# JingInAI/Quantize

Hardware: AMD Instinct MI355X
Metric: quant-conv2d images/sec at batch 256 (ResNet-50, W8A8) (higher is better)
Workload: dtype int8

## Files before the change

### quantize_amd/capi.py

```python
import contextlib
import ctypes
import os

from . import loader

_lib = None

QE_OK = 0
QE_ERR_UNSUPPORTED = 7
DTYPES = {"uint8": 0, "int8": 1, "int16": 2, "int32": 3, "int64": 4,
          "float16": 5, "float32": 6, "float64": 7}

ACTS = {None: 0, "none": 0, "gelu": 1}


class QeConvShape(ctypes.Structure):
    _fields_ = [(n, ctypes.c_int32) for n in ("N", "IC", "H", "W", "OC", "KH", "KW", "stride", "padding")]


class QeQParam(ctypes.Structure):
    _fields_ = [("data", ctypes.c_void_p), ("n_bits", ctypes.c_int32), ("sign", ctypes.c_int32),
                ("scale", ctypes.c_void_p), ("zero", ctypes.c_void_p), ("n_param", ctypes.c_int32)]


class QeRequant(ctypes.Structure):
    _fields_ = [("scale", ctypes.c_void_p), ("zero", ctypes.c_void_p), ("n_param", ctypes.c_int32),
                ("qmin", ctypes.c_float), ("qmax", ctypes.c_float), ("n_bits", ctypes.c_int32), ("sign", ctypes.c_int32)]


class QeError(RuntimeError):
    pass


_vp, _i32, _i64, _sz, _f32, _str = (ctypes.c_void_p, ctypes.c_int, ctypes.c_int64, ctypes.c_size_t, ctypes.c_float,
                                    ctypes.c_char_p)
_pq, _ps, _pr, _ppc = ctypes.POINTER(QeQParam), ctypes.POINTER(QeConvShape), ctypes.POINTER(QeRequant), ctypes.POINTER(_vp)
_attn = [_vp, _vp, _vp, _vp, _i32, _i32, _i32, _i32, _i32, _i64, _i64, _i64, _i64, _i64, _i64, _f32]

PROTOTYPES = {
    "qe_error_string": (_str, [_i32]),
    "qe_last_hip_error": (_i32, []),
    "qe_version": (_str, []),
    "qe_target_arch": (_str, []),
    "qe_packed_nbytes": (_i64, [_i64, _i32]),
    "qe_tpack": (_i32, [_vp, _i32, _i64, _i32, _i32, _vp, _vp, _vp]),
    "qe_tunpack": (_i32, [_vp, _i64, _i32, _i32, _vp, _vp]),
    "qe_quantize_pack": (_i32, [_vp, _i64, _vp, _vp, _i32, _i64, _f32, _f32, _i32, _i32, _vp, _vp, _vp]),
    "qe_quantize_pack_act": (_i32, [_vp, _i64, _i32, _vp, _vp, _i32, _i64, _f32, _f32, _i32, _i32, _vp, _vp, _vp, _vp]),
    "qe_quantize_patchify": (_i32, [_vp, _i32, _i32, _i32, _i32, _i32, _vp, _vp, _i32, _f32, _f32, _i32, _i32, _vp, _vp, _vp]),
    "qe_global_avgpool": (_i32, [_vp, _i64, _i32, _vp, _vp]),
    "qe_maxpool2d_codes": (_i32, [_vp, _i32, _i32, _i32, _i32, _i32, _i32, _i32, _vp, _vp]),
    "qe_quantconv2d_path": (_i32, [_ps, _pq, _pq]),
    "qe_quantconv2d_workspace_bytes": (_sz, [_ps, _i32, _i32]),
    "qe_quantconv2d": (_i32, [_pq, _pq, _vp, _ps, _vp, _vp, _sz, _vp]),
    "qe_conv_prepared_bytes": (_sz, [_ps, _i32, _i32]),
    "qe_conv_prepared_layout": (ctypes.c_uint64, [_ps, _i32, _i32]),
    "qe_conv_prepare": (_i32, [_pq, _vp, _ps, _i32, _vp, _sz, _vp]),
    "qe_quantconv2d_prepared_workspace_bytes": (_sz, [_ps, _i32, _i32]),
    "qe_quantconv2d_prepared": (_i32, [_pq, _pq, _vp, _ps, _vp, _sz, _vp, _vp, _sz, _vp]),
    "qe_quantconv2d_requant_path": (_i32, [_ps, _pq, _pq, _pr]),
    "qe_quantconv2d_requant_workspace_bytes": (_sz, [_ps, _pq, _pq, _pr]),
    "qe_quantconv2d_requant_prepared": (_i32, [_pq, _pq, _vp, _ps, _vp, _sz, _pr, _vp, _vp, _vp, _sz, _vp]),
    "qe_quantconv2d_residual_path": (_i32, [_ps, _pq, _pq, _pr]),
    "qe_quantconv2d_residual_workspace_bytes": (_sz, [_ps, _pq, _pq, _pr]),
    "qe_quantconv2d_residual_prepared": (_i32, [_pq, _pq, _vp, _ps, _vp, _sz, _vp, _vp, _pr, _vp, _vp, _vp, _sz, _vp]),
    "qe_quantconv2d_float_input": (_i32, [_vp, _pq, _vp, _ps, _vp, _vp]),
    "qe_quantconv2d_float_input_path": (_i32, [_ps, _pq]),
    "qe_quantconv2d_float_input_workspace_bytes": (_sz, [_ps, _i32]),
    "qe_quantconv2d_float_input_ws": (_i32, [_vp, _pq, _vp, _ps, _vp, _vp, _sz, _vp]),
    "qe_conv_f32_prepare": (_i32, [_pq, _vp, _ps, _vp, _sz, _vp]),
    "qe_quantconv2d_float_input_prepared": (_i32, [_vp, _pq, _vp, _ps, _vp, _sz, _vp, _vp]),
    "qe_quantlinear": (_i32, [_pq, _pq, _vp, _i64, _i32, _i32, _vp, _vp]),
    "qe_quantlinear_path": (_i32, [_pq, _pq, _i64, _i32, _i32]),
    "qe_quantlinear_form": (_i32, [_pq, _pq, _i64, _i32, _i32, _i32]),
    "qe_quantlinear_float_input": (_i32, [_vp, _pq, _vp, _i64, _i32, _i32, _vp, _vp]),
    "qe_quantlinear_float_input_path": (_i32, [_vp, _pq, _i64, _i32, _i32]),
    "qe_quantlinear_requant_path": (_i32, [_pq, _pq, _i64, _i32, _i32, _pr, _vp]),
    "qe_quantlinear_requant_workspace_bytes": (_sz, [_pq, _pq, _i64, _i32, _i32, _pr, _vp]),
    "qe_quantlinear_requant": (_i32, [_pq, _pq, _vp, _i64, _i32, _i32, _i32, _pr, _vp, _vp, _vp, _sz, _vp]),
    "qe_quantlinear_residual_path": (_i32, [_pq, _pq, _i64, _i32, _i32]),
    "qe_quantlinear_residual_workspace_bytes": (_sz, [_pq, _pq, _i64, _i32, _i32]),
    "qe_quantlinear_residual": (_i32, [_pq, _pq, _vp, _i64, _i32, _i32, _vp, _vp, _vp, _sz, _vp]),
    "qe_quantlinear_float_input_residual_path": (_i32, [_vp, _pq, _i64, _i32, _i32]),
    "qe_quantlinear_float_input_residual_workspace_bytes": (_sz, [_vp, _pq, _i64, _i32, _i32]),
    "qe_quantlinear_float_input_residual": (_i32, [_vp, _pq, _vp, _i64, _i32, _i32, _vp, _vp, _vp, _sz, _vp]),
    "qe_layernorm_quantize_pack_path": (_i32, [_i64, _i32, _i32, _pr, _ppc]),
    "qe_layernorm_quantize_pack_workspace_bytes": (_sz, [_i64, _i32, _i32, _pr, _ppc, _vp]),
    "qe_layernorm_quantize_pack": (_i32, [_vp, _i64, _i32, _vp, _vp, _f32, _i32, _pr, _ppc, _vp, _vp, _vp, _sz, _vp]),
    "qe_attention_path": (_i32, [_i32, _i32, _i32, _i32]),
    "qe_attention": (_i32, _attn + [_vp]),
    "qe_attention_masked_path": (_i32, [_i32, _i32, _i32, _i32, _i32, _i32, _i32]),
    "qe_attention_masked": (_i32, _attn + [_vp, _i64, _i64, _vp, _i32, _vp]),
}
SYMBOLS = sorted(PROTOTYPES)
DEBUG_PROTOTYPES = {
    "qe_debug_reload_env": (None, []),
    "qe_debug_set_stamp_buffer": (None, [_vp]),
}


def lib():
    global _lib
    if _lib is not None:
        return _lib
    path = os.environ.get("QE_LIB") or loader.lib_path()
    if not os.path.exists(path):
        raise ImportError("libqe_hip.so not built: run `python -m quantize_amd.build`. No fallback exists.")
    L = ctypes.CDLL(path)
    for table in (PROTOTYPES, DEBUG_PROTOTYPES):
        for name, (restype, argtypes) in table.items():
            f = getattr(L, name)
            f.restype, f.argtypes = restype, argtypes
    _lib = L
    return L


def check(rc):
    if rc != QE_OK:
        L = lib()
        msg = L.qe_error_string(rc).decode()
        if rc == 5:
            msg += " (hipError_t %d)" % L.qe_last_hip_error()
        raise QeError(msg)


def _stream(stream=None):
    import torch
    s = torch.cuda.current_stream() if stream is None else stream
    return ctypes.c_void_p(s.cuda_stream)


def _ptr(t):
    return None if t is None else t.data_ptr()


def _ws(need, dev):
    import torch
    return torch.empty(need, dtype=torch.uint8, device=dev) if need else None


def _status(status, dev):
    import torch
    return torch.zeros(1, dtype=torch.int32, device=dev) if status is None else status


def _prep(t):
    return (t.data_ptr(), t.numel()) if t is not None and t.numel() else (None, 0)


def packed_nbytes(n, n_bits):
    return int(lib().qe_packed_nbytes(int(n), int(n_bits)))


def tpack(x, n_bits, sign, out=None, status=None, stream=None):
    import torch
    assert x.is_cuda and x.is_contiguous()
    n = x.numel()
    if out is None:
        out = torch.empty(packed_nbytes(n, n_bits), dtype=torch.uint8, device=x.device)
    status = _status(status, x.device)
    check(lib().qe_tpack(x.data_ptr(), DTYPES[str(x.dtype).replace("torch.", "")], n, int(n_bits),
                         1 if sign else 0, out.data_ptr(), status.data_ptr(), _stream(stream)))
    return out, status


def tunpack(packed, n, n_bits, sign, out=None, stream=None):
    import torch
    assert packed.is_cuda and packed.is_contiguous() and packed.dtype == torch.uint8
    if out is None:
        out = torch.empty(n, dtype=torch.int8 if sign else torch.uint8, device=packed.device)
    check(lib().qe_tunpack(packed.data_ptr(), int(n), int(n_bits), 1 if sign else 0, out.data_ptr(),
                           _stream(stream)))
    return out


def conv_shape(N, IC, H, W, OC, KH, KW, stride, padding):
    return QeConvShape(int(N), int(IC), int(H), int(W), int(OC), int(KH), int(KW), int(stride), int(padding))


def out_hw(sh):
# ... 413 lines not shown
```

### quantize_amd/csrc/qe_api.hip

```cpp
#include "qe_common.h"
#include "qe_conv_plan.hpp"

#include <atomic>
#include <cstring>
#include <mutex>
#include <string>
#include <utility>
#include <vector>
#include <unistd.h>

extern char **environ;

namespace qe {

thread_local int g_last_hip_error = 0;

namespace {
struct EnvSnapshot {
    std::vector<std::pair<std::string, std::string>> kv;
};
std::atomic<EnvSnapshot *> g_env{nullptr};
std::mutex g_env_mutex;
EnvSnapshot *take_env_snapshot()
{
// ... 31 lines not shown
                               uint8_t *codes, int32_t *status, hipStream_t s);

static int check_shape(const qe_conv_shape *sh)
{
    if (sh == nullptr) return QE_ERR_ARG;
    if (sh->N < 0 || sh->IC <= 0 || sh->H <= 0 || sh->W <= 0 || sh->OC < 0 || sh->KH <= 0 || sh->KW <= 0 ||
        sh->stride <= 0 || sh->padding < 0)
        return QE_ERR_ARG;
    return QE_OK;
}

static int check_nparam(const qe_qparam *x, const qe_qparam *w, const qe_conv_shape *sh)
{
    if (x != nullptr && !(x->n_param == 1 || x->n_param >= sh->IC)) return QE_ERR_ARG;
    if (!(w->n_param == 1 || w->n_param >= sh->OC)) return QE_ERR_ARG;
    return QE_OK;
}

static int check_qparam(const qe_qparam *q)
{
    if (q == nullptr || q->data == nullptr || q->scale == nullptr || q->zero == nullptr) return QE_ERR_ARG;
    if (!(q->n_bits > 0 && q->n_bits <= 8)) return QE_ERR_NBITS;
    if (q->n_param < 1) return QE_ERR_ARG;
    return QE_OK;
}

static int check_packed_conv(const qe_conv_shape *sh, const qe_qparam *x, const qe_qparam *w)
{
    int rc = check_shape(sh);
    if (rc != QE_OK) return rc;
    if ((rc = check_qparam(x)) != QE_OK) return rc;
    if ((rc = check_qparam(w)) != QE_OK) return rc;
    return check_nparam(x, w, sh);
}

}

extern "C" const char *qe_error_string(int status)
{
    switch (status) {
        case QE_OK: return "ok";
        case QE_ERR_NBITS: return "n_bits must be in the range (0, 8]";
        case QE_ERR_RANGE: return "The input tensor is out of range.";
        case QE_ERR_DTYPE: return "unsupported element type";
        case QE_ERR_ARG: return "invalid argument";
        case QE_ERR_HIP: return "HIP runtime error";
        case QE_ERR_WORKSPACE: return "workspace too small";
        case QE_ERR_UNSUPPORTED: return "problem shape not supported by the gfx950 kernels";
        default: return "unknown error";
    }
}

extern "C" int qe_last_hip_error(void) { return qe::g_last_hip_error; }

extern "C" void qe_debug_reload_env(void)
{
    std::lock_guard<std::mutex> lock(qe::g_env_mutex);
    qe::g_env.store(qe::take_env_snapshot(), std::memory_order_release);
}
extern "C" const char *qe_version(void) { return "quantize_amd 0.1.0"; }
extern "C" const char *qe_target_arch(void) { return "gfx950"; }

namespace qe {
static ConvPlan plan_bits(const qe_conv_shape *sh, int x_bits, int w_bits)
{
    qe_qparam x{}, w{};
    x.n_bits = x_bits; x.n_param = 1;
    w.n_bits = w_bits; w.n_param = 1;
    return plan_conv({sh, &x, &w});
}
static size_t scratch_bytes(const ConvPlan &p) { return (p.m.total - p.m.prep_total + 255) / 256 * 256; }
}

extern "C" size_t qe_quantconv2d_workspace_bytes(const qe_conv_shape *shape, int x_bits, int w_bits)
{
    if (qe::check_shape(shape) != QE_OK) return 0;
    return qe::plan_bits(shape, x_bits, w_bits).m.total;
}

extern "C" int qe_quantconv2d_path(const qe_conv_shape *shape, const qe_qparam *x, const qe_qparam *w)
{
    if (qe::check_shape(shape) != QE_OK || x == nullptr || w == nullptr) return 0;
    return qe::plan_conv({shape, x, w}).route != qe::ConvRoute::Generic ? 1 : 0;
}

extern "C" int qe_quantconv2d(const qe_qparam *x, const qe_qparam *w, const float *bias,
                              const qe_conv_shape *shape, float *out,
                              void *workspace, size_t workspace_bytes, qe_stream_t stream)
{
    using namespace qe;
    const int rc = check_packed_conv(shape, x, w);
    if (rc != QE_OK) return rc;
    if (out == nullptr) return QE_ERR_ARG;
    hipStream_t s = static_cast<hipStream_t>(stream);
    const ConvPlan p = plan_conv({shape, x, w, reinterpret_cast<uintptr_t>(out)});
    if (p.route == ConvRoute::Generic) return launch_conv_generic(true, x->data, x, w, bias, shape, out, s);
    return launch_conv_mfma(p, x, w, bias, shape, out, workspace, workspace_bytes, nullptr, 0, false, s, nullptr, nullptr);
}

extern "C" size_t qe_conv_prepared_bytes(const qe_conv_shape *shape, int x_bits, int w_bits)
{
    if (qe::check_shape(shape) != QE_OK) return 0;
    return qe::plan_prepared(shape, x_bits, w_bits).prep_total;
}

extern "C" uint64_t qe_conv_prepared_layout(const qe_conv_shape *shape, int x_bits, int w_bits)
{
    if (qe::check_shape(shape) != QE_OK) return 0;
    return qe::prepared_layout(qe::plan_prepared(shape, x_bits, w_bits), shape);
}

extern "C" size_t qe_quantconv2d_prepared_workspace_bytes(const qe_conv_shape *shape, int x_bits, int w_bits)
{
    if (qe::check_shape(shape) != QE_OK) return 0;
    const qe::ConvPlan p = qe::plan_bits(shape, x_bits, w_bits);
    return p.m.total - p.m.prep_total;
}

extern "C" int qe_conv_prepare(const qe_qparam *w, const float *bias, const qe_conv_shape *shape, int x_bits,
                               void *prepared, size_t prepared_bytes, qe_stream_t stream)
{
    using namespace qe;
    int rc = check_shape(shape);
    if (rc != QE_OK) return rc;
    if ((rc = check_qparam(w)) != QE_OK) return rc;
    if ((rc = check_nparam(nullptr, w, shape)) != QE_OK) return rc;
    if (!(x_bits > 0 && x_bits <= 8)) return QE_ERR_NBITS;
    return prepare_conv_tables(plan_prepared(shape, x_bits, w->n_bits), w, bias, shape, prepared, prepared_bytes,
                               static_cast<hipStream_t>(stream));
}

extern "C" int qe_quantconv2d_prepared(const qe_qparam *x, const qe_qparam *w, const float *bias,
                                       const qe_conv_shape *shape, const void *prepared, size_t prepared_bytes,
                                       float *out, void *workspace, size_t workspace_bytes, qe_stream_t stream)
{
    using namespace qe;
    const int rc = check_packed_conv(shape, x, w);
    if (rc != QE_OK) return rc;
    if (out == nullptr) return QE_ERR_ARG;
    hipStream_t s = static_cast<hipStream_t>(stream);
    const ConvPlan p = plan_conv({shape, x, w, reinterpret_cast<uintptr_t>(out)});
    if (p.route == ConvRoute::Generic)
        return launch_conv_generic(true, x->data, x, w, bias, shape, out, s);
    return launch_conv_mfma(p, x, w, bias, shape, out, workspace, workspace_bytes, prepared, prepared_bytes, true, s, nullptr,
                            nullptr);
}

static int check_requant(const qe_requant *rq)
{
    if (rq == nullptr || rq->scale == nullptr || rq->zero == nullptr) return QE_ERR_ARG;
    if (!(rq->n_bits > 0 && rq->n_bits <= 8)) return QE_ERR_NBITS;
    if (rq->n_param < 1) return QE_ERR_ARG;
    return QE_OK;
}

static qe::ConvPlan plan_requant(const qe_conv_shape *shape, const qe_qparam *x, const qe_qparam *w, const qe_requant *rq,
                                 const uint8_t *out)
{
    qe::ConvRequest r{shape, x, w};
    r.rq_out = reinterpret_cast<uintptr_t>(out);
    r.rq_bits = rq->n_bits;
    r.rq_n_param = rq->n_param;
    return qe::plan_conv(r);
}

extern "C" int qe_quantconv2d_requant_path(const qe_conv_shape *shape, const qe_qparam *x, const qe_qparam *w, const qe_requant *rq)
// ... 271 lines not shown
```

### quantize_amd/csrc/qe_conv_flatd.hip

```cpp
#include "qe_conv_mfma_kernel.hpp"
#include "qe_conv_plan.hpp"

#include <utility>

namespace qe {

struct FlatdArgs {
    const uint8_t *x;
    const uint8_t *w;
    const float *x_scale, *x_zero, *w_scale, *w_zero, *bias;
    int x_sign, w_sign, w_per_tensor;
    float *out;
    int N, IC, OC, P;
    int tiles_per_image;
    int n_pix_tiles, n_oc_tiles, chunk;
    uint8_t *rq_out;
    const float *rq_scale, *rq_zero;
    float rq_qmin, rq_qmax, rq_lo, rq_hi;
    unsigned rq_offset;
    int32_t *rq_status;
};

constexpr int FD_RING_DEFAULT = 3;

// ... 227 lines not shown
        for (int t = 0; t < NT; ++t) {
            const int v = sxacc[t] + __shfl_xor(sxacc[t], 32);
            if (h == 0) sxp[32 * t + col] = v;
        }
    }
    __syncthreads();
    if constexpr (RQ) {
        uint8_t *bp = smem + wave * (32 * 49 * 4);
        const int oc0 = ot * FD_MT + wave * 32;
        RqConst rqc = rq_setup(a);
        rqc.slow = __builtin_amdgcn_readfirstlane(rqc.slow);
        rqc.chk = __builtin_amdgcn_readfirstlane(rqc.chk);
        bool bad = false;
        const bool fast = rq_fast_ok(rqc) && __builtin_amdgcn_ballot_w64(!rq_bounded(alpha, cst, bia, zwp)) == 0ull;
#pragma unroll
        for (int gi = 0; gi < 4; ++gi) {
            const bool img = n0 + gi < a.N;
#pragma unroll
            for (int tt = 0; tt < 2; ++tt) {
#pragma unroll
                for (int r = 0; r < 16; r += 2) {
                    const int pxl = 32 * tt + (r & 3) + 8 * (r >> 2) + 4 * h;
                    float f0 = (float)acc[2 * gi + tt][r] + cst, f1 = (float)acc[2 * gi + tt][r + 1] + cst;
                    if (need_sx) {
                        f0 = fmaf(-zwp, (float)sxp[64 * gi + pxl], f0);
                        f1 = fmaf(-zwp, (float)sxp[64 * gi + pxl + 1], f1);
                    }
                    const float y0 = fmaf(alpha, f0, bia), y1 = fmaf(alpha, f1, bia);
                    float c0, c1;
                    if (fast) {
                        const v2f c2 = rq_fast2(rqc, v2f{y0, y1});
                        c0 = c2.x; c1 = c2.y;
                    } else {
                        bool b0 = false, b1 = false;
                        c0 = rq_value(rqc, y0, b0);
                        c1 = rq_value(rqc, y1, b1);
                        bad |= img && oc < a.OC && ((b0 && pxl < P) || (b1 && pxl + 1 < P));
                    }
                    if (pxl < P) bp[col * P + pxl] = (uint8_t)(unsigned)c0;
                    if (pxl + 1 < P) bp[col * P + pxl + 1] = (uint8_t)(unsigned)c1;
                }
            }
            if (img && oc0 + 32 <= a.OC) {
                uint8_t *dst = a.rq_out + ((int64_t)(n0 + gi) * a.OC + oc0) * P;
#pragma unroll
                for (int k = 0; k < 2; ++k) {
                    const uint4 d4 = *reinterpret_cast<const uint4 *>(bp + 16 * (64 * k + lane));
                    if (64 * k + lane < 98) *reinterpret_cast<uint4 *>(dst + 16 * (64 * k + lane)) = d4;
                }
            }
        }
        rq_report(a, bad);
    } else {
        float *patch = reinterpret_cast<float *>(smem) + wave * (32 * 49);
        const int oc0 = ot * FD_MT + wave * 32;
        const int vrows = min(32, a.OC - oc0);
        const int nfl = vrows > 0 ? vrows * P : 0;
        const bool vec_ok = (reinterpret_cast<uintptr_t>(a.out) & 15) == 0;
#pragma unroll
        for (int gi = 0; gi < 4; ++gi) {
#pragma unroll
            for (int tt = 0; tt < 2; ++tt) {
#pragma unroll
                for (int r = 0; r < 16; ++r) {
                    const int pxl = 32 * tt + (r & 3) + 8 * (r >> 2) + 4 * h;
                    float f = (float)acc[2 * gi + tt][r] + cst;
                    if (need_sx) f = fmaf(-zwp, (float)sxp[64 * gi + pxl], f);
                    if (pxl < P) patch[col * P + pxl] = fmaf(alpha, f, bia);
                }
            }
            __builtin_amdgcn_s_waitcnt(0xc07f);
            if (n0 + gi < a.N) {
                float *dst = a.out + ((int64_t)(n0 + gi) * a.OC + oc0) * P;
                for (int i = lane; 4 * i < nfl; i += 64) {
                    if (vec_ok && 4 * i + 4 <= nfl) *reinterpret_cast<float4 *>(dst + 4 * i) = *reinterpret_cast<const float4 *>(patch + 4 * i);
                    else for (int b = 4 * i; b < nfl && b < 4 * i + 4; ++b) dst[b] = patch[b];
                }
            }
            __builtin_amdgcn_s_waitcnt(0xc07f);
        }
    }
}

int launch_flatd(const ConvPlan &p, const qe_qparam *x, const qe_qparam *w, const float *bias, float *out, hipStream_t s,
                 const RequantHost *rq)
{
    const qe_conv_shape *sh = &p.run;
    FlatdArgs a;
    a.rq_out = nullptr; a.rq_scale = nullptr; a.rq_zero = nullptr; a.rq_status = nullptr;
    a.rq_qmin = a.rq_qmax = a.rq_lo = a.rq_hi = 0.0f; a.rq_offset = 0;
    if (rq != nullptr) {
        a.rq_out = rq->out; a.rq_scale = rq->scale; a.rq_zero = rq->zero;
        a.rq_qmin = rq->qmin; a.rq_qmax = rq->qmax; a.rq_status = rq->status;
        a.rq_offset = rq->sign ? 128u : 0u;
        a.rq_lo = rq->sign ? -128.0f : 0.0f; a.rq_hi = rq->sign ? 127.0f : 255.0f;
    }
    a.x = static_cast<const uint8_t *>(x->data); a.w = static_cast<const uint8_t *>(w->data);
    a.x_scale = x->scale; a.x_zero = x->zero; a.w_scale = w->scale; a.w_zero = w->zero; a.bias = bias;
    a.x_sign = x->sign; a.w_sign = w->sign; a.w_per_tensor = (w->n_param == 1);
    a.out = out; a.N = sh->N; a.IC = sh->IC; a.OC = sh->OC; a.P = sh->H * sh->W;
    a.n_oc_tiles = p.n_oc_tiles;
    a.tiles_per_image = p.tiles_h;
    a.n_pix_tiles = p.n_pix_tiles;
    a.chunk = p.chunk;
    const int64_t blocks = p.blocks;
#define QE_FD_LAUNCH(WV, RQ)                                                                                                \
    do {                                                                                                                    \
        static const bool ok_ = hipFuncSetAttribute(reinterpret_cast<const void *>(&conv_flatd_kernel<3, WV, RQ>),          \
                                                    hipFuncAttributeMaxDynamicSharedMemorySize, FdGeom<3, WV>::LDS) == hipSuccess; \
        (void)ok_;                                                                                                          \
        constexpr size_t lds_ = FdGeom<3, WV>::LDS;                                                                         \
        hipLaunchKernelGGL((conv_flatd_kernel<3, WV, RQ>), dim3((unsigned)blocks), dim3(64 * WV), lds_, s, a);              \
    } while (0)
    if (rq != nullptr) {
        if (p.fd_w8) QE_FD_LAUNCH(8, true); else QE_FD_LAUNCH(4, true);
    } else {
        if (p.fd_w8) QE_FD_LAUNCH(8, false); else QE_FD_LAUNCH(4, false);
    }
#undef QE_FD_LAUNCH
    QE_LAUNCH_CHECK();
    return QE_OK;
}

}
```

### quantize_amd/csrc/qe_conv_plan.hip

```cpp
#include "qe_conv_plan.hpp"
#include "qe_conv_mfma_kernel.hpp"

#include <algorithm>
#include <cstdlib>

namespace qe {

static int knob(const char *name, int dflt)
{
    const char *e = env_get(name);
    return e ? atoi(e) : dflt;
}

static size_t align_up(size_t v, size_t a) { return (v + a - 1) / a * a; }

static const int kNiw[3][3] = {{7, 4, 2}, {4, 2, 1}, {2, 1, 0}};
static const int kWN[3] = {1, 2, 4};

static MfmaPlan make_plan8(const qe_conv_shape *sh, int w_bits, bool x4 = false)
{
    MfmaPlan p;
    p.OH = (sh->H + 2 * sh->padding - sh->KH) / sh->stride + 1;
    p.OW = (sh->W + 2 * sh->padding - sh->KW) / sh->stride + 1;
    p.KK = sh->KH * sh->KW;
// ... 221 lines not shown
    return p;
}

MfmaPlan plan_prepared(const qe_conv_shape *sh, int x_bits, int w_bits)
{
    qe_conv_shape s1 = *sh;
    const int64_t img = (int64_t)sh->IC * sh->H * sh->W;
    s1.N = img >= 64 ? 1 : (int)((64 + img - 1) / img);
    return make_plan(&s1, x_bits, w_bits);
}

uint64_t prepared_layout(const MfmaPlan &p, const qe_conv_shape *sh)
{
    if (!p.ok || p.prep_total == 0) return 0;
    uint64_t h = 1469598103934665603ull;
    auto mix = [&](uint64_t v) { h = (h ^ v) * 1099511628211ull; };
    mix(p.smallic ? 1 : 0); mix((uint64_t)p.OCP); mix((uint64_t)p.NG); mix((uint64_t)p.KK); mix((uint64_t)sh->KH); mix((uint64_t)sh->KW);
    mix((uint64_t)sh->IC); mix((uint64_t)sh->OC); mix((uint64_t)p.prep_total); mix((uint64_t)p.ep_off); mix((uint64_t)p.ws_off);
    return h | 1ull;
}

struct PwrFit {
    int tw = 0, ks = 0, groups = 1;
    bool s2 = false;
};

static bool pwr_plan(const qe_conv_shape *sh, const qe_qparam *x, const qe_qparam *w, uintptr_t xa, PwrFit *pl)
{
    const int mode = knob("QE_PWR", 2);
    if (mode == 0) return false;
    if (sh->KH != 1 || sh->KW != 1 || sh->padding != 0 || (sh->stride != 1 && sh->stride != 2)) return false;
    if (x->n_bits != 8 || w->n_bits != 8 || x->n_param != 1) return false;
    if (sh->IC != 64 && sh->IC != 128 && sh->IC != 256) return false;
    if (sh->OC % 32 != 0 || sh->OC < 128 || sh->N < 1) return false;
    const bool s2 = sh->stride == 2;
    if (s2 && ((sh->H & 1) || (sh->W & 7) || sh->W > 64 || knob("QE_PWR_S2", 1) == 0)) return false;
    const int OH = s2 ? sh->H / 2 : sh->H, OW = s2 ? sh->W / 2 : sh->W;
    const int64_t P = (int64_t)OH * OW;
    const int tw = (P % 224 == 0) ? 224 : ((P % 196 == 0) ? 196 : 0);
    if (tw == 0) return false;
    if (s2 && (tw % OW != 0 || tw / OW > 8)) return false;
    if (mode == 1 && !s2 && P != tw) return false;
    if ((int64_t)sh->N * sh->IC * sh->H * sh->W < 16 || (int64_t)sh->OC * P >= (1ll << 29) || (int64_t)sh->IC * sh->H * sh->W >= (1ll << 31)) return false;
    if ((reinterpret_cast<uintptr_t>(w->data) & 15) != 0 || (xa & (s2 ? 7 : 3)) != 0) return false;
    if ((reinterpret_cast<uintptr_t>(w->scale) & 3) != 0) return false;
    const int ks = sh->IC / 32;
    const int waves = ks == 8 ? 8 : 4;
    if (sh->OC < 64 * waves) return false;
    const int strips = sh->OC / 32;
    const int g = knob("QE_PWR_GROUPS", 0);
    pl->tw = tw; pl->ks = ks; pl->groups = (g >= 1 && strips % g == 0) ? g : 1; pl->s2 = s2;
    return true;
}

static int pwr7_plan(const qe_conv_shape *sh, const qe_qparam *x, const qe_qparam *w, uintptr_t xa, int *groups)
{
    if (knob("QE_PWR", 2) == 0 || knob("QE_PWR7", 1) == 0) return 0;
    if (sh->KH != 1 || sh->KW != 1 || sh->stride != 1 || sh->padding != 0 || sh->H * sh->W != 49) return 0;
    if (x->n_bits != 8 || w->n_bits != 8 || x->n_param != 1) return 0;
    if (sh->IC != 128 && sh->IC != 256 && sh->IC != 512) return 0;
    const int gi = sh->IC == 512 ? 2 : 4;
    if (sh->OC % 32 != 0 || sh->OC < 512 || sh->N < gi || sh->N % gi != 0) return 0;
    if ((int64_t)sh->N * sh->IC * 49 >= (1ll << 31) || (int64_t)sh->OC * 49 >= (1ll << 29)) return 0;
    if ((reinterpret_cast<uintptr_t>(w->data) & 15) != 0 || (xa & 15) != 0) return 0;
    const int tiles = sh->N / gi, strips = sh->OC / 32;
    int g = 1;
    while (tiles * g < kNumCU && strips % (2 * g) == 0 && strips / (2 * g) >= 8) g *= 2;
    const int ge = knob("QE_PWR_GROUPS", 0);
    *groups = (ge >= 1 && strips % ge == 0) ? ge : g;
    return gi;
}

static bool flatd_plan(const qe_conv_shape *sh, const qe_qparam *x, const qe_qparam *w, uintptr_t xa)
{
    if (sh->KH != 1 || sh->KW != 1 || sh->stride != 1 || sh->padding != 0) return false;
    if (x->n_bits != 8 || w->n_bits != 8 || x->n_param != 1) return false;
    if (sh->IC % FD_CK != 0 || sh->IC < 2 * FD_CK || sh->OC < 1 || sh->N < 1) return false;
    const int64_t P = (int64_t)sh->H * sh->W;
    if ((int64_t)sh->N * sh->IC * P < 16 || (int64_t)sh->OC * P >= (1ll << 29) || (int64_t)sh->IC * P >= (1ll << 31)) return false;
    if ((reinterpret_cast<uintptr_t>(w->data) & 15) != 0) return false;
    return P == 49 && sh->OC % 4 == 0 && (xa & 15) == 0;
}

static int64_t block_map(ConvPlan &p, int64_t n_units, int per_image, int64_t per_tile, bool knob_ok = true)
{
    const int64_t per_xcd = (n_units + 7) / 8;
    const int64_t k = knob_ok ? (int64_t)knob("QE_CHUNK_IMAGES", 1 << 20) * per_image : per_xcd;
    p.chunk = (int)std::max<int64_t>(1, std::min<int64_t>(per_xcd, k));
    const int64_t runs = (n_units + p.chunk - 1) / p.chunk;
    return (runs + 7) / 8 * p.chunk * 8 * per_tile;
}

static bool plan_rq_patch(const MfmaPlan &m, const ConvRequest &r)
{
    if (m.flat || m.flatg || m.ws || m.GI != 1 || (m.OH * m.OW) % 4 != 0 || (m.TH * m.OW) % 4 != 0) return false;
    if ((r.rq_out & 3) != 0 || knob("QE_RQ_PATCH", 1) == 0) return false;
    const int wm = m.cfg == 0 ? 4 : (m.cfg == 1 ? 2 : 1);
    const int kkt = m.KK == 1 ? 1 : ((m.KK == 9 && r.sh->KW == 3) ? 9 : 0);
    if (m.sm2) return mfma_has_patch(MfKind::Sm2, wm, m.niw, kkt, m.NS);
    return mfma_has_patch(m.smallic ? MfKind::Stem : MfKind::Halo, wm, m.niw, kkt, m.NS);
}

static void plan_mfma_launch(ConvPlan &p, const ConvRequest &r, bool rq)
{
    const MfmaPlan &m = p.m;
    const qe_conv_shape *sh = &p.run;
    p.tiles_h = (m.OH + m.TH - 1) / m.TH;
    p.n_pix_tiles = ((sh->N + m.GI - 1) / m.GI) * p.tiles_h;
    p.n_oc_tiles = m.OCP / m.MT;
    if (m.flatg) {
        p.tiles_h = 1;
        p.n_pix_tiles = (sh->N + m.GI - 1) / m.GI;
    } else if (m.flat) {
        p.tiles_h = m.IHT;
        p.n_pix_tiles = sh->N * p.tiles_h;
    }
    p.blocks = block_map(p, p.n_pix_tiles, p.tiles_h, p.n_oc_tiles);
    auto clipped_lo = [](int pad, int stride, int O) { return std::min(O, (pad + stride - 1) / stride); };
    auto clipped_hi = [](int I, int pad, int K, int stride, int O) {
        const int full_last = (I + pad - K) >= 0 ? (I + pad - K) / stride : -1;
        return std::max(0, std::min(O, O - 1 - full_last));
    };
    p.n_top = clipped_lo(sh->padding, sh->stride, m.OH);
    p.n_bot = clipped_hi(sh->H, sh->padding, sh->KH, sh->stride, m.OH);
    p.n_lft = clipped_lo(sh->padding, sh->stride, m.OW);
    p.n_rgt = clipped_hi(sh->W, sh->padding, sh->KW, sh->stride, m.OW);

    if (m.flat || m.flatg) {
        p.lds = m.lds;
        if (rq) {
            p.ptab_off = (int)align_up(m.lds, 16);
            p.lds = p.ptab_off + (m.flatg ? (size_t)m.GI * m.MT * sh->H * sh->W : (size_t)m.MT * 32 * m.ni);
        }
        return;
    }
    p.rq_patch = rq && plan_rq_patch(m, r);
    const size_t stage_bytes = p.rq_patch ? std::max(m.lds, (size_t)32 * 1024) : m.lds;
    size_t lds_e = stage_bytes;
    const size_t tab = (size_t)m.MT * (sh->KH + 1) * (sh->KW + 1) * sizeof(int);
    const size_t off = align_up(stage_bytes, 16);
    if (off + tab <= (size_t)(m.sm2 ? MF_MAX_LDS_SM2 : MF_MAX_LDS)) { p.ptab_off = (int)off; lds_e = off + tab; }
    const int ncls = (1 + p.n_top + p.n_bot) * (1 + p.n_lft + p.n_rgt);
    p.ctab = p.ptab_off != 0 && p.n_top + p.n_bot < m.OH && p.n_lft + p.n_rgt < m.OW && ncls <= (sh->KH + 1) * (sh->KW + 1) &&
             knob("QE_CTAB", 1) != 0;
    const int units = m.GI * m.IHT * ((sh->W + 3) / 4);
    p.split = units <= 64 ? 4 : (units <= 128 ? 2 : 1);
    p.lds = (m.ws && !p.ctab) ? m.lds : lds_e;
}

ConvPlan plan_conv(const ConvRequest &r)
{
    ConvPlan p;
    const qe_conv_shape *sh = r.sh;
    p.OH = (sh->H + 2 * sh->padding - sh->KH) / sh->stride + 1;
    p.OW = (sh->W + 2 * sh->padding - sh->KW) / sh->stride + 1;
    if (p.OH > 0 && p.OW > 0) p.y_bytes = align_up((size_t)sh->N * sh->OC * p.OH * p.OW * sizeof(float), 256);
    p.m = make_plan(sh, r.x->n_bits, r.w->n_bits);
    const MfmaPlan &m = p.m;
    if (r.x->n_param != 1 || !m.ok) return p;
    p.run = m.sub ? dense_shape(sh) : *sh;
    const qe_conv_shape *rs = &p.run;

    qe_qparam xr = *r.x;
    uintptr_t xa = reinterpret_cast<uintptr_t>(r.x->data);
    if (m.sub_x4 || m.expand) { xr.n_bits = 8; xr.sign = 1; }
    if (m.sub || m.expand) xa = 0;
    if (m.sub_x4) {
        p.pre = PrePass::SubX4;
        p.pre_blocks = ((int64_t)sh->N * sh->IC * rs->H * ((rs->W + 7) / 8) + 255) / 256;
    } else if (m.sub) {
        const int64_t n_planes = (int64_t)sh->N * sh->IC;
        const int nq = (rs->W + 7) / 8;
        int log_nq = 0;
        while ((1 << log_nq) < nq) ++log_nq;
        const int units2 = rs->H << log_nq;
        if (sh->stride == 2 && (sh->H % 2) == 0 && (1 << log_nq) == nq && 16 * nq <= 2 * sh->W && units2 <= 256 &&
            knob("QE_SUB2", 1) != 0) {
            int log_up = 3;
            while ((1 << log_up) < units2) ++log_up;
            p.pre = PrePass::Sub2;
            p.sub2_log_nq = log_nq;
            p.sub2_log_up = log_up;
            const int ppb = (256 >> log_up) * 4;
            p.pre_blocks = (n_planes + ppb - 1) / ppb;
        } else {
            const bool wide = sh->stride == 2 && (sh->W % 4) == 0 && sh->W >= 16;
            const int units = rs->H * ((rs->W + (wide ? 7 : 3)) / (wide ? 8 : 4));
            const int ppb = units >= 1024 ? 1 : 1024 / units;
            p.pre = wide ? PrePass::SubWide : PrePass::SubNarrow;
            p.pre_blocks = (n_planes + ppb - 1) / ppb;
        }
    }
    if (p.pre_blocks > 0x7fffffffLL) return p;

    PwrFit pf;
    int g7 = 1;
    if (r.residual) {
        if (r.rq_bits != 0 && (r.rq_bits != 8 || r.rq_n_param != 1)) return p;
        if (m.sub || m.expand || rs->stride != 1) return p;
        if (pwr_plan(rs, &xr, r.w, xa, &pf)) p.route = ConvRoute::Pwr;
        else if (rs->IC == 512 && (p.pwr7_gi = pwr7_plan(rs, &xr, r.w, xa, &g7)) != 0) p.route = ConvRoute::Pwr7;
        else return p;
        p.fused = true;
    } else {
        const bool rq = r.rq_bits > 0;
        if (rq) {
            if (r.rq_bits != 8 || r.rq_n_param != 1) return p;
            if (m.flat || m.flatg) {
                const size_t patch = m.flatg ? (size_t)m.GI * m.MT * rs->H * rs->W : (size_t)m.MT * 32 * m.ni;
                if (align_up(m.lds, 16) + patch > (size_t)MF_MAX_LDS) return p;
            }
            p.fused = true;
        }
        const bool pwr_ok = rq ? (r.rq_out & 15) == 0 && knob("QE_PWR_RQ", 1) != 0 : true;
        const bool fd_ok = flatd_plan(rs, &xr, r.w, xa) && knob("QE_FLATD", 1) != 0 &&
                           (!rq || (rs->OC % 32 == 0 && (r.rq_out & 15) == 0 && knob("QE_FLATD_RQ", 1) != 0));
        if (pwr_ok && pwr_plan(rs, &xr, r.w, xa, &pf)) p.route = ConvRoute::Pwr;
        else if (pwr_ok && (rq || (r.out & 15) == 0) && (p.pwr7_gi = pwr7_plan(rs, &xr, r.w, xa, &g7)) != 0) p.route = ConvRoute::Pwr7;
        else if (fd_ok) p.route = ConvRoute::Flatd;
        else p.route = ConvRoute::Mfma;
    }

    if (p.route == ConvRoute::Pwr) {
        p.pwr_tw = pf.tw; p.pwr_ks = pf.ks; p.pwr_groups = pf.groups; p.pwr_s2 = pf.s2;
        const int64_t P = pf.s2 ? (int64_t)(rs->H / 2) * (rs->W / 2) : (int64_t)rs->H * rs->W;
        p.tiles_h = (int)(P / pf.tw);
        p.n_pix_tiles = rs->N * p.tiles_h;
        p.blocks = block_map(p, p.n_pix_tiles, p.tiles_h, pf.groups);
    } else if (p.route == ConvRoute::Pwr7) {
        p.pwr_groups = g7;
        p.tiles_h = 1;
        p.n_pix_tiles = rs->N / p.pwr7_gi;
        p.blocks = block_map(p, p.n_pix_tiles, 1, g7, false);
    } else if (p.route == ConvRoute::Flatd) {
        const char *e8 = env_get("QE_FLATD8");
        p.fd_w8 = e8 ? atoi(e8) != 0 && rs->OC > 128 : rs->OC >= 1024;
        const int MT = p.fd_w8 ? 256 : 128;
        p.n_oc_tiles = (rs->OC + MT - 1) / MT;
        p.tiles_h = 1;
        p.n_pix_tiles = (rs->N + 3) / 4;
        p.blocks = block_map(p, p.n_pix_tiles, p.tiles_h, p.n_oc_tiles);
    } else {
        plan_mfma_launch(p, r, p.fused);
    }
    if (p.blocks > 0x7fffffffLL) { p.route = ConvRoute::Generic; p.fused = false; }
    return p;
}

}
```

### quantize_amd/csrc/qe_conv_plan.hpp

```cpp
#pragma once
#include "qe_common.h"

namespace qe {

struct RequantHost {
    uint8_t *out;
    const float *scale, *zero;
    int n_param;
    float qmin, qmax;
    int n_bits, sign;
    int32_t *status;
};

constexpr int FD_CK = 64;

struct MfmaPlan {
    bool ok = false;
    int cfg = 0;
    int MT = 0, OCP = 0, NCH = 0, NG = 0, KK = 0, OH = 0, OW = 0;
    int TH = 0, ni = 0, niw = 0, IHT = 0, IWP = 0, ROWMUL = 1, COLMUL = 1;
    bool smallic = false;
    int GI = 1, NS = 1;
    bool flat = false, wraw = false, ws = false, s2 = false, sm2 = false;
    bool expand = false;
    bool x4 = false;
    size_t xe_off = 0;
    bool flatg = false;
    bool sub = false;
    bool sub_x4 = false;
    size_t sub_off = 0;
    size_t lds = 0;
    size_t wt_bytes = 0, ep_off = 0, ws_off = 0, total = 0;
    size_t prep_total = 0;
};

enum class ConvRoute { Generic, Pwr, Pwr7, Flatd, Mfma };
enum class PrePass { None, SubX4, Sub2, SubWide, SubNarrow };

struct ConvRequest {
    const qe_conv_shape *sh;
    const qe_qparam *x, *w;
    uintptr_t out = 0;
    uintptr_t rq_out = 0;
    int rq_bits = 0;
    int rq_n_param = 1;
    bool residual = false;
};

struct ConvPlan {
    ConvRoute route = ConvRoute::Generic;
    bool fused = false;
    int OH = 0, OW = 0;
    size_t y_bytes = 0;
    MfmaPlan m;
    qe_conv_shape run{};

    PrePass pre = PrePass::None;
    int64_t pre_blocks = 0;
    int sub2_log_up = 0, sub2_log_nq = 0;

    int64_t blocks = 0;
    int chunk = 1, n_pix_tiles = 0, n_oc_tiles = 0, tiles_h = 0;
    size_t lds = 0;

    int pwr_tw = 0, pwr_ks = 0, pwr_groups = 1, pwr7_gi = 0;
    bool pwr_s2 = false;
    bool fd_w8 = false;
    bool rq_patch = false;
    bool ctab = false;
    int ptab_off = 0;
    int n_top = 0, n_bot = 0, n_lft = 0, n_rgt = 0;
    int split = 1;
};

ConvPlan plan_conv(const ConvRequest &rq);
MfmaPlan plan_prepared(const qe_conv_shape *sh, int x_bits, int w_bits);
uint64_t prepared_layout(const MfmaPlan &p, const qe_conv_shape *sh);

int launch_conv_mfma(const ConvPlan &p, const qe_qparam *x, const qe_qparam *w, const float *bias, const qe_conv_shape *sh,
                     float *out, void *workspace, size_t workspace_bytes, const void *prepared, size_t prepared_bytes,
                     bool use_prepared, hipStream_t s, const RequantHost *rq, const float *res);
int prepare_conv_tables(const MfmaPlan &p, const qe_qparam *w, const float *bias, const qe_conv_shape *sh, void *prepared,
                        size_t prepared_bytes, hipStream_t s);
int launch_pwr(const ConvPlan &p, const qe_qparam *x, const qe_qparam *w, const float *bias, float *out, hipStream_t s,
               const RequantHost *rq, const float *res);
int launch_flatd(const ConvPlan &p, const qe_qparam *x, const qe_qparam *w, const float *bias, float *out, hipStream_t s,
                 const RequantHost *rq);

enum class F32Kernel {
    Stem4x1x7, Stem2x2x4, Stem2x2x7,
    M4x1x4, M4x1x4S2, M4x1x7, M4x1x7S2, M2x2x2, M2x2x2S2, M2x2x4, M2x2x4S2
};

struct F32Plan {
    bool ok = false;
    F32Kernel kernel = F32Kernel::M4x1x7;
    bool stem = false;
    int OCP = 0, NG = 0, KK = 0, OH = 0, OW = 0;
    int TH = 0, GI = 1, IHT = 0, IWP = 0, ROWMUL = 1, COLMUL = 1;
    int64_t blocks = 0;
    int chunk = 1, n_pix_tiles = 0, n_oc_tiles = 0, tiles_h = 0;
    size_t lds = 0;
    size_t ep_off = 0, total = 0;
};

F32Plan plan_conv_f32(const qe_conv_shape *sh);
int prepare_conv_f32(const F32Plan &p, const qe_qparam *w, const float *bias, const qe_conv_shape *sh, void *prepared,
                     size_t prepared_bytes, hipStream_t s);
int launch_conv_f32(const F32Plan &p, const float *x, const qe_conv_shape *sh, const void *prepared, size_t prepared_bytes,
                    float *out, hipStream_t s);

}
```

Before: 61880.

## Add specialized flat-direct 1x1 conv kernel for 14x14 spatial layers

Adds a dedicated int8 MFMA kernel for 1x1 stride-1 convolutions with 196 output pixels and IC>=512. Each block covers one whole image's 196 pixels and a 128-wide output-channel tile, staging activations and weights through a 3-deep LDS ring via global_load_lds and reading them with transposing ds_read_b64_tr_b8. Stores go through LDS patches so global writes are coalesced. The planner routes eligible non-requant shapes here ahead of the existing flatd path, and a debug entry point exposes the plan. The risks are the heavy register footprint from seven 32x32 accumulators and the padding of 196 pixels to 224.

```diff
diff --git a/quantize_amd/capi.py b/quantize_amd/capi.py
--- a/quantize_amd/capi.py
+++ b/quantize_amd/capi.py
@@ -96,6 +96,7 @@
 DEBUG_PROTOTYPES = {
     "qe_debug_reload_env": (None, []),
     "qe_debug_set_stamp_buffer": (None, [_vp]),
+    "qe_debug_conv_plan": (_i32, [_ps, _pq, _pq, _vp, _i32, _i32, ctypes.POINTER(_i64)]),
 }
 
 
diff --git a/quantize_amd/csrc/qe_api.hip b/quantize_amd/csrc/qe_api.hip
--- a/quantize_amd/csrc/qe_api.hip
+++ b/quantize_amd/csrc/qe_api.hip
@@ -137,6 +137,24 @@
 {
     if (qe::check_shape(shape) != QE_OK || x == nullptr || w == nullptr) return 0;
     return qe::plan_conv({shape, x, w}).route != qe::ConvRoute::Generic ? 1 : 0;
+}
+
+extern "C" int qe_debug_conv_plan(const qe_conv_shape *shape, const qe_qparam *x, const qe_qparam *w, const void *out, int rq_bits,
+                                  int residual, int64_t *info)
+{
+    if (qe::check_shape(shape) != QE_OK || x == nullptr || w == nullptr) return -1;
+    qe::ConvRequest r{shape, x, w, reinterpret_cast<uintptr_t>(out)};
+    r.rq_bits = rq_bits;
+    r.residual = residual != 0;
+    const qe::ConvPlan p = qe::plan_conv(r);
+    if (info != nullptr) { info[0] = p.blocks; info[1] = p.n_pix_tiles; info[2] = p.n_oc_tiles; info[3] = p.tiles_h; }
+    switch (p.route) {
+        case qe::ConvRoute::Generic: return 0;
+        case qe::ConvRoute::Pwr: return 1;
+        case qe::ConvRoute::Pwr7: return 2;
+        case qe::ConvRoute::Flatd: return p.fd_196 ? 5 : 3;
+        default: return 4;
+    }
 }
 
 extern "C" int qe_quantconv2d(const qe_qparam *x, const qe_qparam *w, const float *bias,
diff --git a/quantize_amd/csrc/qe_conv_flatd.hip b/quantize_amd/csrc/qe_conv_flatd.hip
--- a/quantize_amd/csrc/qe_conv_flatd.hip
+++ b/quantize_amd/csrc/qe_conv_flatd.hip
@@ -333,6 +333,222 @@
     }
 }
 
+struct Fd196Geom {
+    static constexpr int RING = 3;
+    static constexpr int TW = 196, NT = 7, NTP = 224;
+    static constexpr int RS = 224;
+    static constexpr int XBYTES = FD_CK * RS;
+    static constexpr int WBYTES = 128 * FD_CK;
+    static constexpr int STAGE = XBYTES + WBYTES;
+    static constexpr int XI = XBYTES / 256 / 4;
+    static constexpr int RING_BYTES = RING * STAGE;
+    static constexpr int PATCH = 16 * TW * 4;
+    static constexpr int NPIECE = (16 * TW / 4 + 63) / 64;
+    static constexpr int LDS = RING_BYTES + 4 * NTP * 4 ;
+    static_assert(4 * PATCH + 1024 <= RING_BYTES, "store patches live in the ring");
+};
+
+__device__ __forceinline__ void fd_reads_wide7(uint32_t tr_addr, uint32_t wf_addr, v4i &wf, v2i (&lo)[7], v2i (&hi)[7])
+{
+    asm volatile(
+        "ds_read_b128 %0, %16\n\t"
+        "ds_read_b64_tr_b8 %1, %15 offset:0\n\t"
+        "ds_read_b64_tr_b8 %8, %15 offset:1792\n\t"
+        "ds_read_b64_tr_b8 %2, %15 offset:32\n\t"
+        "ds_read_b64_tr_b8 %9, %15 offset:1824\n\t"
+        "ds_read_b64_tr_b8 %3, %15 offset:64\n\t"
+        "ds_read_b64_tr_b8 %10, %15 offset:1856\n\t"
+        "ds_read_b64_tr_b8 %4, %15 offset:96\n\t"
+        "ds_read_b64_tr_b8 %11, %15 offset:1888\n\t"
+        "ds_read_b64_tr_b8 %5, %15 offset:128\n\t"
+        "ds_read_b64_tr_b8 %12, %15 offset:1920\n\t"
+        "ds_read_b64_tr_b8 %6, %15 offset:160\n\t"
+        "ds_read_b64_tr_b8 %13, %15 offset:1952\n\t"
+        "ds_read_b64_tr_b8 %7, %15 offset:192\n\t"
+        "ds_read_b64_tr_b8 %14, %15 offset:1984\n\t"
+        "s_waitcnt lgkmcnt(0)"
+        : "=&v"(wf), "=&v"(lo[0]), "=&v"(lo[1]), "=&v"(lo[2]), "=&v"(lo[3]), "=&v"(lo[4]), "=&v"(lo[5]), "=&v"(lo[6]), "=&v"(hi[0]), "=&v"(hi[1]), "=&v"(hi[2]), "=&v"(hi[3]), "=&v"(hi[4]), "=&v"(hi[5]), "=&v"(hi[6])
+        : "v"(tr_addr), "v"(wf_addr));
+}
+__device__ __forceinline__ void fd196_patch_read(uint32_t addr, v4i (&o)[13])
+{
+    asm volatile("ds_read_b128 %0, %13\n\tds_read_b128 %1, %13 offset:1024\n\tds_read_b128 %2, %13 offset:2048\n\t"
+                 "ds_read_b128 %3, %13 offset:3072\n\tds_read_b128 %4, %13 offset:4096\n\tds_read_b128 %5, %13 offset:5120\n\t"
+                 "ds_read_b128 %6, %13 offset:6144\n\tds_read_b128 %7, %13 offset:7168\n\tds_read_b128 %8, %13 offset:8192\n\t"
+                 "ds_read_b128 %9, %13 offset:9216\n\tds_read_b128 %10, %13 offset:10240\n\tds_read_b128 %11, %13 offset:11264\n\t"
+                 "ds_read_b128 %12, %13 offset:12288\n\ts_waitcnt lgkmcnt(0)"
+                 : "=&v"(o[0]), "=&v"(o[1]), "=&v"(o[2]), "=&v"(o[3]), "=&v"(o[4]), "=&v"(o[5]), "=&v"(o[6]), "=&v"(o[7]), "=&v"(o[8]),
+                   "=&v"(o[9]), "=&v"(o[10]), "=&v"(o[11]), "=&v"(o[12])
+                 : "v"(addr) : "memory");
+}
+
+__global__ __launch_bounds__(256, 2) void conv_flatd196_kernel(const FlatdArgs a)
+{
+    using G = Fd196Geom;
+    constexpr int AHEAD = G::RING - 1;
+    extern __shared__ __attribute__((aligned(16))) uint8_t smem[];
+
+    const int tid = threadIdx.x, lane = tid & 63;
+    const int wave = __builtin_amdgcn_readfirstlane(tid >> 6);
+    const int col = lane & 31, h = lane >> 5;
+    constexpr int P = G::TW;
+
+    int pt, ot;
+    {
+        const int bid = blockIdx.x;
+        const int idx = bid >> 3;
+        const int j = idx / a.n_oc_tiles;
+        ot = idx - j * a.n_oc_tiles;
+        const int c = j / a.chunk;
+        pt = (c * 8 + (bid & 7)) * a.chunk + (j - c * a.chunk);
+    }
+    if (pt >= a.n_pix_tiles) return;
+    const int n0 = pt;
+
+    const int oc = ot * 128 + wave * 32 + col;
+    const int occ = oc < a.OC ? oc : a.OC - 1;
+    const float sw = a.w_per_tensor ? a.w_scale[0] : a.w_scale[occ];
+    const float zwp = (a.w_per_tensor ? a.w_zero[0] : a.w_zero[occ]) - (a.w_sign ? 0.0f : 128.0f);
+    const float alpha = a.x_scale[0] * sw;
+    const float bia = a.bias ? a.bias[occ] : 0.0f;
+    const float zxp = a.x_zero[0] - (a.x_sign ? 0.0f : 128.0f);
+
+    uint32_t xoff[G::XI];
+#pragma unroll
+    for (int i = 0; i < G::XI; ++i) {
+        const int d = 64 * (wave + 4 * i) + lane;
+        const int c = d / 56, j = d - 56 * c;
+        xoff[i] = (uint32_t)c * (uint32_t)P + 4u * (uint32_t)(j < 48 ? j : 48);
+    }
+    const uint8_t *xtile = a.x + (int64_t)n0 * a.IC * P;
+    const uint8_t *pw[2];
+#pragma unroll
+    for (int i = 0; i < 2; ++i) {
+        const int e = tid + 256 * i;
+        const int r = e >> 2, sl = e & 3;
+        const int orow = ot * 128 + r < a.OC ? ot * 128 + r : a.OC - 1;
+        pw[i] = a.w + (int64_t)orow * a.IC + 16 * (sl ^ ((r >> 2) & 3));
+    }
+    const int64_t x_step = (int64_t)FD_CK * P;
+    const int n_stages = a.IC / FD_CK;
+    auto issue = [&](int s) __attribute__((always_inline)) {
+        uint8_t *buf = smem + (s % G::RING) * G::STAGE;
+        const uint8_t *xs = xtile + s * x_step;
+#pragma unroll
+        for (int i = 0; i < G::XI; ++i)
+            __builtin_amdgcn_global_load_lds((const __attribute__((address_space(1))) void *)(xs + xoff[i]),
+                                             (__attribute__((address_space(3))) void *)(buf + 256 * (wave + 4 * i)), 4, 0, 0);
+#pragma unroll
+        for (int i = 0; i < 2; ++i)
+            __builtin_amdgcn_global_load_lds((const __attribute__((address_space(1))) void *)(pw[i] + s * FD_CK),
+                                             (__attribute__((address_space(3))) void *)(buf + G::XBYTES + (256 * i + 64 * wave) * 16), 16, 0, 0);
+    };
+
+    issue(0);
+    issue(1);
+
+    const bool need_sx = __builtin_amdgcn_ballot_w64(oc < a.OC && zwp != 0.0f) != 0ull;
+    int *sxp = reinterpret_cast<int *>(smem + G::RING_BYTES) + wave * G::NTP;
+
+    v16i acc[G::NT];
+#pragma unroll
+    for (int t = 0; t < G::NT; ++t)
+#pragma unroll
+        for (int r = 0; r < 16; ++r) acc[t][r] = 0;
+    int swacc = 0;
+    int sxacc[G::NT];
+#pragma unroll
+    for (int t = 0; t < G::NT; ++t) sxacc[t] = 0;
+
+    const int i16 = lane & 15;
+    const uint32_t smem_lds = (uint32_t)(uintptr_t)(__attribute__((address_space(3))) uint8_t *)smem;
+    const uint32_t tr_b = (uint32_t)((16 * h + (i16 >> 1)) * G::RS + 16 * ((lane >> 4) & 1) + 8 * (i16 & 1));
+    const int wf_base = G::XBYTES + (wave * 32 + col) * FD_CK;
+    const int wswz = (col >> 2) & 3;
+
+    auto main_loop = [&](auto sx_tag) __attribute__((always_inline)) {
+        constexpr bool SX = decltype(sx_tag)::value;
+        for (int s = 0; s < n_stages; ++s) {
+            if (s + 1 < n_stages) __builtin_amdgcn_s_waitcnt(0x0f70 | ((G::XI + 2) & 15) | (((G::XI + 2) >> 4) << 14));
+            else __builtin_amdgcn_s_waitcnt(0x0f70);
+            __builtin_amdgcn_s_barrier();
+            if (s + AHEAD < n_stages) issue(s + AHEAD);
+            const uint32_t xb = smem_lds + (uint32_t)((s % G::RING) * G::STAGE);
+#pragma unroll
+            for (int k = 0; k < 2; ++k) {
+                v2i lo[G::NT], hi[G::NT];
+                v4i wf;
+                const uint32_t wfa = xb + (uint32_t)(wf_base + 16 * ((2 * k + h) ^ wswz));
+                fd_reads_wide7(xb + tr_b + k * 32 * G::RS, wfa, wf, lo, hi);
+#pragma unroll
+                for (int j = 0; j < 4; ++j) {
+                    wf[j] ^= (int)0x80808080;
+                    swacc = __builtin_amdgcn_sdot4(wf[j], 0x01010101, swacc, false);
+                }
+#pragma unroll
+                for (int t = 0; t < G::NT; ++t) {
+                    v4i xf = {lo[t][0], lo[t][1], hi[t][0], hi[t][1]};
+#pragma unroll
+                    for (int j = 0; j < 4; ++j) xf[j] ^= (int)0x80808080;
+                    if constexpr (SX) {
+#pragma unroll
+                        for (int j = 0; j < 4; ++j) sxacc[t] = __builtin_amdgcn_sdot4(xf[j], 0x01010101, sxacc[t], false);
+                    }
+                    acc[t] = __builtin_amdgcn_mfma_i32_32x32x32_i8(xf, wf, acc[t], 0, 0, 0);
+                }
+            }
+        }
+    };
+    if (need_sx) main_loop(std::true_type{}); else main_loop(std::false_type{});
+
+    const int sw_sum = swacc + __shfl_xor(swacc, 32);
+    const float cst = fmaf((float)a.IC * zxp, zwp, -zxp * (float)sw_sum);
+    if (need_sx) {
+#pragma unroll
+        for (int t = 0; t < G::NT; ++t) {
+            const int v = sxacc[t] + __shfl_xor(sxacc[t], 32);
+            if (h == 0) sxp[32 * t + col] = v;
+        }
+    }
+    __syncthreads();
+    const uint32_t patch = smem_lds + (uint32_t)(wave * G::PATCH);
+    const uint32_t pwr = patch + (uint32_t)((col & 15) * G::TW * 4 + 16 * h);
+    const int oc0 = ot * 128 + wave * 32;
+#pragma unroll
+    for (int hf = 0; hf < 2; ++hf) {
+        if ((col >> 4) == hf) {
+#pragma unroll
+            for (int t = 0; t < G::NT; ++t) {
+#pragma unroll
+                for (int gq = 0; gq < (t == 6 ? 1 : 4); ++gq) {
+                    float v[4];
+#pragma unroll
+                    for (int j = 0; j < 4; ++j) {
+                        float f = (float)acc[t][4 * gq + j] + cst;
+                        if (need_sx) f = fmaf(-zwp, (float)sxp[32 * t + 8 * gq + 4 * h + j], f);
+                        v[j] = fmaf(alpha, f, bia);
+                    }
+                    if (t < 6 || h == 0) fd_patch_write(pwr + (uint32_t)((32 * t + 8 * gq) * 4), v[0], v[1], v[2], v[3]);
+                }
+            }
+        }
+        fd_lds_drain();
+        v4i o[G::NPIECE];
+        fd196_patch_read(patch + 16u * (uint32_t)lane, o);
+        const int rows = min(16, a.OC - (oc0 + 16 * hf));
+        float *dst = a.out + ((int64_t)n0 * a.OC + oc0 + 16 * hf) * P + 4 * lane;
+        if (rows == 16) {
+#pragma unroll
+            for (int it = 0; it < G::NPIECE - 1; ++it) *reinterpret_cast<v4i *>(dst + 256 * it) = o[it];
+            if (lane < 16) *reinterpret_cast<v4i *>(dst + 256 * (G::NPIECE - 1)) = o[G::NPIECE - 1];
+        } else if (rows > 0) {
+#pragma unroll
+            for (int it = 0; it < G::NPIECE; ++it)
+                if (64 * it + lane < rows * 49) *reinterpret_cast<v4i *>(dst + 256 * it) = o[it];
+        }
+    }
+}
+
 int launch_flatd(const ConvPlan &p, const qe_qparam *x, const qe_qparam *w, const float *bias, float *out, hipStream_t s,
                  const RequantHost *rq)
 {
@@ -355,6 +571,14 @@
     a.n_pix_tiles = p.n_pix_tiles;
     a.chunk = p.chunk;
     const int64_t blocks = p.blocks;
+    if (p.fd_196) {
+        static const bool ok_ = hipFuncSetAttribute(reinterpret_cast<const void *>(&conv_flatd196_kernel),
+                                                    hipFuncAttributeMaxDynamicSharedMemorySize, Fd196Geom::LDS) == hipSuccess;
+        (void)ok_;
+        hipLaunchKernelGGL(conv_flatd196_kernel, dim3((unsigned)blocks), dim3(256), (size_t)Fd196Geom::LDS, s, a);
+        QE_LAUNCH_CHECK();
+        return QE_OK;
+    }
 #define QE_FD_LAUNCH(WV, RQ)                                                                                                \
     do {                                                                                                                    \
         static const bool ok_ = hipFuncSetAttribute(reinterpret_cast<const void *>(&conv_flatd_kernel<3, WV, RQ>),          \
diff --git a/quantize_amd/csrc/qe_conv_plan.hip b/quantize_amd/csrc/qe_conv_plan.hip
--- a/quantize_amd/csrc/qe_conv_plan.hip
+++ b/quantize_amd/csrc/qe_conv_plan.hip
@@ -327,6 +327,17 @@
     return P == 49 && sh->OC % 4 == 0 && (xa & 15) == 0;
 }
 
+static bool flatd196_plan(const qe_conv_shape *sh, const qe_qparam *x, const qe_qparam *w, uintptr_t xa, uintptr_t out)
+{
+    if (sh->KH != 1 || sh->KW != 1 || sh->stride != 1 || sh->padding != 0) return false;
+    if (x->n_bits != 8 || w->n_bits != 8 || x->n_param != 1) return false;
+    if (sh->IC % FD_CK != 0 || sh->IC < 512 || sh->OC < 1 || sh->N < 1) return false;
+    const int64_t P = (int64_t)sh->H * sh->W;
+    if (P != 196 || sh->OC % 4 != 0) return false;
+    if ((int64_t)sh->OC * P >= (1ll << 29) || (int64_t)sh->IC * P >= (1ll << 31)) return false;
+    return (xa & 3) == 0 && (reinterpret_cast<uintptr_t>(w->data) & 15) == 0 && (out & 15) == 0;
+}
+
 static int64_t block_map(ConvPlan &p, int64_t n_units, int per_image, int64_t per_tile, bool knob_ok = true)
 {
     const int64_t per_xcd = (n_units + 7) / 8;
@@ -460,8 +471,10 @@
         const bool pwr_ok = rq ? (r.rq_out & 15) == 0 && knob("QE_PWR_RQ", 1) != 0 : true;
         const bool fd_ok = flatd_plan(rs, &xr, r.w, xa) && knob("QE_FLATD", 1) != 0 &&
                            (!rq || (rs->OC % 32 == 0 && (r.rq_out & 15) == 0 && knob("QE_FLATD_RQ", 1) != 0));
+        const bool fd196_ok = !rq && !m.sub && knob("QE_FLATD196", 1) != 0 && flatd196_plan(rs, &xr, r.w, xa, r.out);
         if (pwr_ok && pwr_plan(rs, &xr, r.w, xa, &pf)) p.route = ConvRoute::Pwr;
         else if (pwr_ok && (rq || (r.out & 15) == 0) && (p.pwr7_gi = pwr7_plan(rs, &xr, r.w, xa, &g7)) != 0) p.route = ConvRoute::Pwr7;
+        else if (fd196_ok) { p.route = ConvRoute::Flatd; p.fd_196 = true; }
         else if (fd_ok) p.route = ConvRoute::Flatd;
         else p.route = ConvRoute::Mfma;
     }
@@ -477,6 +490,11 @@
         p.tiles_h = 1;
         p.n_pix_tiles = rs->N / p.pwr7_gi;
         p.blocks = block_map(p, p.n_pix_tiles, 1, g7, false);
+    } else if (p.route == ConvRoute::Flatd && p.fd_196) {
+        p.n_oc_tiles = (rs->OC + 127) / 128;
+        p.tiles_h = 1;
+        p.n_pix_tiles = rs->N * p.tiles_h;
+        p.blocks = block_map(p, p.n_pix_tiles, p.tiles_h, p.n_oc_tiles);
     } else if (p.route == ConvRoute::Flatd) {
         const char *e8 = env_get("QE_FLATD8");
         p.fd_w8 = e8 ? atoi(e8) != 0 && rs->OC > 128 : rs->OC >= 1024;
diff --git a/quantize_amd/csrc/qe_conv_plan.hpp b/quantize_amd/csrc/qe_conv_plan.hpp
--- a/quantize_amd/csrc/qe_conv_plan.hpp
+++ b/quantize_amd/csrc/qe_conv_plan.hpp
@@ -66,6 +66,7 @@
     int pwr_tw = 0, pwr_ks = 0, pwr_groups = 1, pwr7_gi = 0;
     bool pwr_s2 = false;
     bool fd_w8 = false;
+    bool fd_196 = false;
     bool rq_patch = false;
     bool ctab = false;
     int ptab_off = 0;
```

Result: no change. 62120 (median of 5 runs) (+0.4%).
